# kontera-technologies/redis-bloomfilter

Measured on AMD Instinct MI355X. Metric: keys/sec (insert, include?) per GPU and whole node; % of HBM random-access roofline, higher is better.
Workload: dtype u32

## Files before the change

### redis-bloomfilter_amd/csrc/bf_api.cpp

```cpp
#include "bfhip.h"
#include "bf_host.h"
#include "bf_multi.h"
#include "bf_device.h"

#include <sched.h>

#include <algorithm>
#include <atomic>
#include <cmath>
#include <condition_variable>
#include <functional>
#include <thread>
#include <cstdio>
#include <cstdlib>
#include <cstring>
#include <mutex>
#include <string>
#include <vector>

#define BFHIP_VERSION_STR "bfhip 0.1.0 (gfx950; redis-bloomfilter 1.1.2 ruby-driver layout)"

namespace {

thread_local std::string g_create_error;
// ... 262 lines not shown

int check_keys_args(bf_handle* h, const void* keys, const uint64_t* offsets, uint64_t n) {
    if (!h) return BF_EINVAL;
    if (n == 0) return BF_OK;
    if (!offsets) return set_err(h, BF_EINVAL, "offsets is NULL");
    if (!keys && offsets[n] != offsets[0]) return set_err(h, BF_EINVAL, "key_bytes is NULL");
    return BF_OK;
}

bool binned_pays(const bf_handle* h, uint32_t mode, double probes) {
    if (mode == 0) return false;
    return mode == 1 || (h->dev_bytes >= (64ull << 20) && probes * 128.0 > kBinnedCostRatio * (double)h->dev_bytes);
}

bool use_binned(const bf_handle* h, uint64_t n, bool include, BfBinPlan* plan) {
    if (h->shards > 1 || h->engine != BF_ENGINE_RUBY) return false;
    return binned_pays(h, include ? h->include_binned_mode : h->binned_mode, (double)n * (double)h->k) &&
           bf_binned_plan(h->dev_bytes, n, h->k, h->bin_region_log2, include, plan);
}

int ensure_scratch(bf_handle* h, uint64_t bytes) {
    if (bytes <= h->bin_scratch_cap) return BF_OK;
    (void)hipDeviceSynchronize();
    if (h->d_bin_scratch) (void)hipFree(h->d_bin_scratch);
    h->d_bin_scratch = nullptr;
    h->bin_scratch_cap = 0;
    const uint64_t cap = round_up(bytes, 16ull << 20);
    HIPCHK(h, hipMalloc(&h->d_bin_scratch, cap));
    h->bin_scratch_cap = cap;
    return BF_OK;
}

const char* op_kernel_name(BfOp op) {
    switch (op) {
        case BF_OP_INDEXES: return "bf_keys_kernel<INDEXES>";
        case BF_OP_INCLUDE: return "bf_keys_kernel<INCLUDE>";
        case BF_OP_INSERT: return "bf_keys_kernel<INSERT>";
        case BF_OP_INSERT_FLAGS: return "bf_keys_kernel<INSERT_FLAGS>";
        default: return "bf_keys_kernel<ROUTE>";
    }
}

int launch_op(bf_handle* h, BfOp op, const uint8_t* k16, const uint64_t* offs, uint64_t bias, uint64_t n,
              uint8_t* out8, uint64_t* out64, uint32_t* flag, hipStream_t s) {
    if (h->engine != BF_ENGINE_RUBY) {
        if (op == BF_OP_INSERT_FLAGS && out8)
            return set_err(h, BF_EINVAL, "per_key_new is not available with a RubyTest hash engine");
        if (op == BF_OP_INSERT_FLAGS) op = BF_OP_INSERT;
        BfMarks* mk = prof_begin(h, s);
        HIPCHK(h, bf_launch_engine(h->engine, op, h->g, k16, offs, bias, n, out8, out64, flag, s));
        bf_mark(mk, s, h->engine == BF_ENGINE_MD5 ? "engine_kernel<MD5>" : "engine_kernel<SHA1>");
// ... 469 lines not shown
int bf_destroy(bf_handle* h) {
    if (!h) return BF_OK;
    if (h->multi) {
        bfm_destroy(h->multi);
        delete h;
        return BF_OK;
    }
    {
        CallScope cs(h);
        DeviceGuard dg(h->device);
        if (h->order_valid) (void)hipEventSynchronize(h->order_ev);
        if (h->stream) (void)hipStreamSynchronize(h->stream);
        free_staging(h);
        if (h->h_small) (void)hipHostFree(h->h_small);
        if (h->d_small) (void)hipFree(h->d_small);
        if (h->g.bits) (void)hipFree(h->g.bits);
        if (h->d_flag) (void)hipFree(h->d_flag);
        if (h->d_scan) (void)hipFree(h->d_scan);
        if (h->h_flag) (void)hipHostFree(h->h_flag);
        if (h->h_key_status) (void)hipHostFree(h->h_key_status);
        if (h->d_tmp_local) (void)hipFree(h->d_tmp_local);
        if (h->d_tmp_owner) (void)hipFree(h->d_tmp_owner);
        if (h->d_cursor) (void)hipFree(h->d_cursor);
        if (h->d_bin_scratch) (void)hipFree(h->d_bin_scratch);
        if (h->d_ans8) (void)hipFree(h->d_ans8);
        if (h->d_seg) (void)hipFree(h->d_seg);
        if (h->d_dirty) (void)hipFree(h->d_dirty);
        (void)prof_harvest(h);
        prof_destroy(h);
        if (h->order_ev) (void)hipEventDestroy(h->order_ev);
        if (h->copy_stream) (void)hipStreamDestroy(h->copy_stream);
        if (h->d2h_stream) (void)hipStreamDestroy(h->d2h_stream);
        if (h->stream) (void)hipStreamDestroy(h->stream);
    }
    delete h;
    return BF_OK;
}

int bf_info(const bf_handle* h, uint64_t* m_bits, uint32_t* k, uint64_t* reach_bits, uint64_t* device_bytes) {
    if (h && h->multi) return bfm_info(h->multi, m_bits, k, reach_bits, device_bytes);
    if (!h) return BF_EINVAL;
    if (m_bits) *m_bits = h->m;
    if (k) *k = h->k;
    if (reach_bits) *reach_bits = h->reach;
    if (device_bytes) *device_bytes = h->dev_bytes;
    return BF_OK;
}
// ... 1428 lines not shown
```

### redis-bloomfilter_amd/csrc/bf_binned.hip

```cpp
#include "bf_device.h"
#include "bfhip.h"

#include <algorithm>
#include <cmath>
#include <cstdlib>

using namespace bfdev;

namespace {
__device__ __forceinline__ void stage_store(uint32_t* p, uint32_t v) { __builtin_nontemporal_store(v, p); }
}

namespace {

constexpr int kTile = 1024;
constexpr int kStageVec = 16384 / 16;
constexpr uint32_t kMaxSup = 256;
constexpr uint32_t kMaxOwners = 256;
constexpr uint32_t kChunkBuckets = 512;
constexpr uint32_t kMaxRel = 9;
constexpr uint32_t kMaxBlocks = 512;
constexpr uint32_t kMaxFrontBlocks = 16384;
constexpr uint32_t kGroupBlocks = 64;
constexpr uint32_t kTileProbes = 12288;
// ... 5 lines not shown
constexpr int kChunkPerLane = kBlockProbes / kTile;
constexpr uint32_t kRunsPerPass = 1024;
constexpr uint32_t kMidBuckets = 128;
constexpr uint32_t kMidParts = 2;
constexpr uint32_t kApplyLanes = 1024;
constexpr uint32_t kPipeLanes = 1024;

__device__ __forceinline__ uint32_t block_excl_scan(uint32_t v, uint32_t* s_w, uint32_t* total) {
    const uint32_t lane = threadIdx.x & 63u, wid = threadIdx.x >> 6, nw = blockDim.x >> 6;
    const uint32_t x = wave_incl_scan(v);
    if (lane == 63u) s_w[wid] = x;
    __syncthreads();
    if (wid == 0) {
        const uint32_t s = wave_incl_scan(lane < nw ? s_w[lane] : 0u);
        if (lane < nw) s_w[lane] = s;
    }
    __syncthreads();
    const uint32_t r = (wid ? s_w[wid - 1] : 0u) + x - v;
    if (total) *total = s_w[nw - 1];
    __syncthreads();
    return r;
}

__device__ __forceinline__ void tile_sha1_words(const uint8_t* keys16, const uint64_t* offsets, uint64_t bias,
                                                uint64_t key0, uint32_t tk, uint32_t* key_status, uint64_t* s_off,
                                                uint4* s_stage, uint4& H0, uint4& H1) {
    auto hash = [&](uint64_t first, uint32_t cnt, uint4& Hd) {
        for_key_tile<kTile, kStageVec>(keys16, offsets, bias, first, cnt, s_off, s_stage, key_status,
            [&](auto staged, uint32_t, const uint32_t* src, uint32_t s, uint32_t L) {
                uint32_t H[5];
                sha1_any<decltype(staged)::value>(src, s, L, H);
                Hd = make_uint4(H[0], H[1], H[2], H[3]);
            });
    };
    hash(key0, tk < (uint32_t)kTile ? tk : kTile, H0);
    if (tk > (uint32_t)kTile) hash(key0 + kTile, tk - kTile, H1);
}

template <bool KEYS, int SLOTS, bool DIG = false>
__device__ __forceinline__ void bin_front_body(BfGeom g, const uint8_t* __restrict__ keys16,
                                                          const uint64_t* __restrict__ offsets, uint64_t bias,
                                                          uint64_t n, uint32_t tile_keys, uint32_t tiles_per_block,
                                                          uint32_t sup_log2, uint32_t nsup,
                                                          uint32_t* __restrict__ level1,
                                                          uint32_t* __restrict__ level1_key,
                                                          uint16_t* __restrict__ stab, uint32_t* __restrict__ gcnt,
                                                          uint8_t* __restrict__ out8) {
    __shared__ uint64_t s_off[kTile + 1];
    __shared__ uint4 s_stage[kStageVec + kStageSlackVec];
    __shared__ uint32_t s_cnt[kMaxSup], s_lbase[kMaxSup], s_gcnt[kMaxSup];
    __shared__ uint32_t s_w[16];
    __shared__ uint32_t s_sorted[kTile * SLOTS];
    __shared__ uint32_t s_key[KEYS ? kTile * SLOTS : 1];
    const uint32_t t = threadIdx.x;
    if (t < kMaxSup) {
        s_cnt[t] = 0;
        s_gcnt[t] = 0;
    }
    __syncthreads();
    const uint32_t k = g.k;
    const uint32_t kpl = tile_keys / kTile;
    const uint64_t smask = (1ull << sup_log2) - 1ull;
    const uint64_t ntiles = (n + tile_keys - 1) / tile_keys;
    const uint64_t tb0 = (uint64_t)blockIdx.x * tiles_per_block;
    const uint64_t tb1 = (tb0 + tiles_per_block < ntiles) ? tb0 + tiles_per_block : ntiles;
    for (uint64_t tile = tb0; tile < tb1; ++tile) {
        const uint64_t key0 = tile * tile_keys;
        const uint32_t tk = (uint32_t)((n - key0) < (uint64_t)tile_keys ? (n - key0) : tile_keys);
        uint4 H0 = make_uint4(0, 0, 0, 0), H1 = make_uint4(0, 0, 0, 0);
        if constexpr (DIG) {
            const uint4* dig = reinterpret_cast<const uint4*>(keys16);
            if (t < tk) H0 = dig[key0 + t];
            if (kTile + t < tk) H1 = dig[key0 + kTile + t];
        } else {
            tile_sha1_words(keys16, offsets, bias, key0, tk, g.key_status, s_off, s_stage, H0, H1);
        }
        const bool live0 = t < tk;
        const bool live1 = kpl == 2 && kTile + t < tk;
        if constexpr (KEYS) {
            if (live0) out8[key0 + t] = 1;
            if (live1) out8[key0 + kTile + t] = 1;
        }
        uint32_t tag[SLOTS], loc[SLOTS];
#pragma unroll
        for (int q = 0; q < SLOTS; ++q) {
            const bool second = kpl == 2 && q >= (int)kTwoKeys;
            const uint32_t i = second ? (uint32_t)q - kTwoKeys : (uint32_t)q;
            const bool live = i < k && (second ? live1 : live0);
            tag[q] = 0xFFFFFFFFu;
            loc[q] = 0;
            if (live) {
                const uint4 H = second ? H1 : H0;
                const uint64_t o = probe_offset(g, H.x, H.y, H.z, H.w, i);
                const uint32_t sb = (uint32_t)(o >> sup_log2);
                tag[q] = (sb << 16) | atomicAdd(s_cnt + sb, 1u);
                loc[q] = (uint32_t)(o & smask);
            }
        }
        __syncthreads();
        const uint32_t c = t < kMaxSup ? s_cnt[t] : 0u;
        const uint32_t ex = block_excl_scan(c, s_w, nullptr);
        if (t <= nsup) stab[(uint64_t)t * ntiles + tile] = (uint16_t)ex;
        if (t < kMaxSup) {
            s_lbase[t] = ex;
            s_gcnt[t] += c;
            s_cnt[t] = 0;
        }
        __syncthreads();
#pragma unroll
        for (int q = 0; q < SLOTS; ++q) {
            if (tag[q] != 0xFFFFFFFFu) {
                const uint32_t d = s_lbase[tag[q] >> 16] + (tag[q] & 0xFFFFu);
                s_sorted[d] = loc[q];
                if constexpr (KEYS) {
                    const bool second = kpl == 2 && q >= (int)kTwoKeys;
                    s_key[d] = (uint32_t)(key0 + (second ? kTile + t : t));
                }
            }
        }
        __syncthreads();
        const uint64_t seg = key0 * k;
        const uint32_t tp = tk * k;
        for (uint32_t j = t; j < tp; j += kTile) {
            stage_store(level1 + seg + j, s_sorted[j]);
            if constexpr (KEYS) level1_key[seg + j] = s_key[j];
        }
    }
    if (t < nsup) gcnt[(uint64_t)blockIdx.x * nsup + t] = s_gcnt[t];
}

template <bool DIG>
__global__ __launch_bounds__(kTile) __attribute__((amdgpu_waves_per_eu(8, 8)))
void bin_front_kernel(BfGeom g, const uint8_t* __restrict__ keys16, const uint64_t* __restrict__ offsets,
                      uint64_t bias, uint64_t n, uint32_t tile_keys, uint32_t tiles_per_block, uint32_t sup_log2,
                      uint32_t nsup, uint32_t* __restrict__ level1, uint32_t* __restrict__ level1_key,
                      uint16_t* __restrict__ stab, uint32_t* __restrict__ gcnt, uint8_t* __restrict__ out8) {
    bin_front_body<false, kSlots, DIG>(g, keys16, offsets, bias, n, tile_keys, tiles_per_block, sup_log2, nsup,
                                       level1, level1_key, stab, gcnt, out8);
}

template <bool KEYS, bool DIG = false>
__global__ __launch_bounds__(kTile) void bin_front_wide_kernel(BfGeom g, const uint8_t* __restrict__ keys16,
                                                               const uint64_t* __restrict__ offsets, uint64_t bias,
                                                               uint64_t n, uint32_t tile_keys,
                                                               uint32_t tiles_per_block, uint32_t sup_log2,
                                                               uint32_t nsup, uint32_t* __restrict__ level1,
                                                               uint32_t* __restrict__ level1_key,
                                                               uint16_t* __restrict__ stab, uint32_t* __restrict__ gcnt,
                                                               uint8_t* __restrict__ out8) {
    bin_front_body<KEYS, kWideSlots, DIG>(g, keys16, offsets, bias, n, tile_keys, tiles_per_block, sup_log2, nsup,
                                          level1, level1_key, stab, gcnt, out8);
}

__global__ __launch_bounds__(kTile) __attribute__((amdgpu_waves_per_eu(8, 8)))
void bin_front_wide_dig_kernel(BfGeom g, const uint8_t* __restrict__ keys16, const uint64_t* __restrict__ offsets,
                               uint64_t bias, uint64_t n, uint32_t tile_keys, uint32_t tiles_per_block,
                               uint32_t sup_log2, uint32_t nsup, uint32_t* __restrict__ level1,
                               uint32_t* __restrict__ level1_key, uint16_t* __restrict__ stab,
                               uint32_t* __restrict__ gcnt, uint8_t* __restrict__ out8) {
    bin_front_body<false, kWideSlots, true>(g, keys16, offsets, bias, n, tile_keys, tiles_per_block, sup_log2, nsup,
                                            level1, level1_key, stab, gcnt, out8);
}

__global__ __launch_bounds__(kTile)
void bin_front_keys_kernel(BfGeom g, const uint8_t* __restrict__ keys16, const uint64_t* __restrict__ offsets,
                           uint64_t bias, uint64_t n, uint32_t tile_keys, uint32_t tiles_per_block, uint32_t sup_log2,
                           uint32_t nsup, uint32_t* __restrict__ level1, uint32_t* __restrict__ level1_key,
                           uint16_t* __restrict__ stab, uint32_t* __restrict__ gcnt, uint8_t* __restrict__ out8) {
    bin_front_body<true, kSlots>(g, keys16, offsets, bias, n, tile_keys, tiles_per_block, sup_log2, nsup, level1,
                                 level1_key, stab, gcnt, out8);
}

template <typename Off, bool KEYS>
__device__ __forceinline__ void bin_front_offsets_body(const Off* __restrict__ local, uint64_t count,
                                                       uint32_t tiles_per_block, uint32_t sup_log2, uint32_t nsup,
                                                       uint32_t* __restrict__ level1,
                                                       uint32_t* __restrict__ level1_key,
                                                       uint16_t* __restrict__ stab, uint32_t* __restrict__ gcnt,
                                                       uint64_t bias, const unsigned long long* __restrict__ wcounts,
                                                       uint32_t wstride, uint64_t wcap, uint64_t limit,
                                                       uint8_t* __restrict__ oob_out) {
    __shared__ uint32_t s_cnt[kMaxSup], s_lbase[kMaxSup], s_gcnt[kMaxSup];
    __shared__ uint32_t s_w[16];
    __shared__ uint32_t s_sorted[kTileProbes];
    __shared__ uint16_t s_key[KEYS ? kTileProbes : 1];
    const uint32_t t = threadIdx.x;
    if (t < kMaxSup) {
        s_cnt[t] = 0;
        s_gcnt[t] = 0;
    }
    __syncthreads();
    const uint64_t smask = (1ull << sup_log2) - 1ull;
    const uint64_t ntiles = (count + kTileProbes - 1) / kTileProbes;
    const bool vec_ok = (reinterpret_cast<uintptr_t>(local) & 15u) == 0;
    static_assert(kTileProbes == kTile * kSlots, "a tile is kSlots entries per lane");
    const uint64_t tb0 = (uint64_t)blockIdx.x * tiles_per_block;
    const uint64_t tb1 = (tb0 + tiles_per_block < ntiles) ? tb0 + tiles_per_block : ntiles;
    for (uint64_t tile = tb0; tile < tb1; ++tile) {
        const uint64_t p0 = tile * kTileProbes;
        uint32_t tp = (uint32_t)((count - p0) < (uint64_t)kTileProbes ? (count - p0) : kTileProbes);
        if (wcounts) {
            const uint64_t w = p0 / wcap, i0 = p0 - w * wcap;
            uint64_t live = wcounts[w * wstride];
            if (live > wcap) live = 0;
// ... 32 lines not shown
        __syncthreads();
        const uint32_t c = t < kMaxSup ? s_cnt[t] : 0u;
        const uint32_t ex = block_excl_scan(c, s_w, nullptr);
        if (t <= nsup) stab[(uint64_t)t * ntiles + tile] = (uint16_t)ex;
        if (t < kMaxSup) {
            s_lbase[t] = ex;
            s_gcnt[t] += c;
            s_cnt[t] = 0;
        }
        __syncthreads();
#pragma unroll
        for (int q = 0; q < kSlots; ++q)
            if (tag[q] != 0xFFFFFFFFu) {
                const uint32_t d = s_lbase[tag[q] >> 16] + (tag[q] & 0xFFFFu);
                s_sorted[d] = loc[q];
                if constexpr (KEYS) s_key[d] = (uint16_t)(t * (uint32_t)kSlots + (uint32_t)q);
            }
        __syncthreads();
        for (uint32_t j = t; j < tp; j += kTile) {
            level1[p0 + j] = s_sorted[j];
            if constexpr (KEYS) level1_key[p0 + j] = (uint32_t)p0 + s_key[j];
        }
    }
    if (t < nsup) gcnt[(uint64_t)blockIdx.x * nsup + t] = s_gcnt[t];
}

template <typename Off>
__global__ __launch_bounds__(kTile) __attribute__((amdgpu_waves_per_eu(8, 8)))
void bin_front_offsets_kernel(const Off* __restrict__ local, uint64_t count, uint32_t tiles_per_block,
                              uint32_t sup_log2, uint32_t nsup, uint32_t* __restrict__ level1,
                              uint16_t* __restrict__ stab, uint32_t* __restrict__ gcnt, uint64_t bias,
                              const unsigned long long* __restrict__ wcounts, uint32_t wstride, uint64_t wcap,
                              uint64_t limit) {
    bin_front_offsets_body<Off, false>(local, count, tiles_per_block, sup_log2, nsup, level1, nullptr, stab, gcnt,
                                       bias, wcounts, wstride, wcap, limit, nullptr);
}

template <typename Off>
__global__ __launch_bounds__(kTile) __attribute__((amdgpu_waves_per_eu(8, 8)))
void bin_front_offsets_keys_kernel(const Off* __restrict__ local, uint64_t count,
                                                                       uint32_t tiles_per_block, uint32_t sup_log2,
                                                                       uint32_t nsup, uint32_t* __restrict__ level1,
                                                                       uint32_t* __restrict__ level1_key,
                                                                       uint16_t* __restrict__ stab,
                                                                       uint32_t* __restrict__ gcnt, uint64_t bias,
                                                                       const unsigned long long* __restrict__ wcounts,
                                                                       uint32_t wstride, uint64_t wcap, uint64_t limit,
                                                                       uint8_t* __restrict__ out8) {
    bin_front_offsets_body<Off, true>(local, count, tiles_per_block, sup_log2, nsup, level1, level1_key, stab, gcnt,
                                      bias, wcounts, wstride, wcap, limit, out8);
}

__global__ __launch_bounds__(kMaxBlocks) void bin_group_sum_kernel(const uint32_t* __restrict__ gcnt,
                                                                   uint32_t nblocks, uint32_t nsup, uint32_t nq,
                                                                   uint32_t* __restrict__ gsum) {
    const uint32_t sb = blockIdx.x;
    for (uint32_t w = threadIdx.x; w < nq * kGroupBlocks; w += kMaxBlocks) {
        uint32_t v = w < nblocks ? gcnt[(uint64_t)w * nsup + sb] : 0u;
#pragma unroll
        for (int off = 32; off > 0; off >>= 1) v += (uint32_t)__shfl_xor((int)v, off);
        if ((w & 63u) == 0) gsum[sb * nq + w / kGroupBlocks] = v;
    }
}

constexpr uint32_t kScanPer = 4;
constexpr uint32_t kScanWindows = 1024 * kScanPer;
constexpr uint32_t kLocalScanPer = 4;
constexpr uint32_t kMaxGroups = 1024 * kLocalScanPer;
constexpr uint32_t kMaxWindows = kMaxSup * kMaxGroups;
__global__ __launch_bounds__(1024) void bin_group_scan_kernel(const uint32_t* __restrict__ gsum, uint32_t N,
                                                              uint32_t* __restrict__ base,
                                                              uint32_t* __restrict__ cb_base,
                                                              uint32_t* __restrict__ cb_window,
                                                              uint32_t* __restrict__ cb_start, uint32_t nq,
                                                              unsigned long long* __restrict__ totals) {
    __shared__ uint32_t s_w[16];
    __shared__ uint32_t s_cb[kScanWindows + 1];
    const uint32_t t = threadIdx.x;
    uint32_t v[kScanPer], cv[kScanPer], sum = 0, csum = 0;
#pragma unroll
    for (uint32_t e = 0; e < kScanPer; ++e) {
        const uint32_t w = kScanPer * t + e;
        v[e] = w < N ? gsum[w] : 0u;
        cv[e] = (v[e] + kBlockProbes - 1) / kBlockProbes;
        sum += v[e];
        csum += cv[e];
    }
    uint32_t total, ctotal;
    uint32_t ex = block_excl_scan(sum, s_w, &total);
    uint32_t cex = block_excl_scan(csum, s_w, &ctotal);
#pragma unroll
    for (uint32_t e = 0; e < kScanPer; ++e) {
        const uint32_t w = kScanPer * t + e;
        if (w < N) {
            base[w] = ex;
            cb_base[w] = cex;
            s_cb[w] = cex;
            if (totals && v[e]) atomicAdd(totals + w / nq, (unsigned long long)v[e]);
        }
        ex += v[e];
        cex += cv[e];
    }
    if (t == 0) {
        base[N] = total;
        cb_base[N] = ctotal;
        s_cb[N] = ctotal;
    }
    __syncthreads();
    for (uint32_t blk = t; blk < ctotal; blk += 1024) {
        uint32_t lo = 0, hi = N - 1;
        while (lo < hi) {
            const uint32_t mid = (lo + hi + 1) >> 1;
            if (s_cb[mid] <= blk) lo = mid; else hi = mid - 1;
        }
        cb_window[blk] = lo;
        cb_start[blk] = base[lo] + (blk - s_cb[lo]) * kBlockProbes;
    }
}

__global__ __launch_bounds__(1024) void bin_scan_local_kernel(const uint32_t* __restrict__ gsum, uint32_t nq,
                                                              uint32_t* __restrict__ base,
                                                              uint32_t* __restrict__ cb_base,
                                                              uint32_t* __restrict__ stot) {
    __shared__ uint32_t s_w[16];
    const uint32_t sb = blockIdx.x, t = threadIdx.x;
    uint32_t v[kLocalScanPer], cv[kLocalScanPer], sum = 0, csum = 0;
#pragma unroll
    for (uint32_t e = 0; e < kLocalScanPer; ++e) {
        const uint32_t q = kLocalScanPer * t + e;
        v[e] = q < nq ? gsum[(uint64_t)sb * nq + q] : 0u;
        cv[e] = (v[e] + kBlockProbes - 1) / kBlockProbes;
        sum += v[e];
        csum += cv[e];
    }
    uint32_t total, ctotal;
    uint32_t ex = block_excl_scan(sum, s_w, &total);
    uint32_t cex = block_excl_scan(csum, s_w, &ctotal);
#pragma unroll
    for (uint32_t e = 0; e < kLocalScanPer; ++e) {
        const uint32_t q = kLocalScanPer * t + e;
// ... 1445 lines not shown
                        const uint32_t ri = (uint32_t)(k4[i] - jbase) - a0;
                        if (((av[u] >> (8 * i)) & 0xFFu) && qa + i >= l0 && qa + i < l1 && ri >= b0 && ri < b1)
                            atomicOr(s_bits + ((ri - b0) >> 5), 1u << (ri & 31u));
                    }
                }
            }
        }
        __syncthreads();
        for (uint32_t i = t; i < pw; i += 1024) {
            const bool edge = (w0 + i == 0) || (w0 + i == nw - 1);
            if (edge) atomicOr(out + w0 + i, s_bits[i]);
            else out[w0 + i] = s_bits[i];
        }
        __syncthreads();
    }
}


uint32_t front_form(uint32_t k) { return k <= kTwoKeys ? 0u : (k <= (uint32_t)kSlots ? 1u : 2u); }
uint32_t front_tile_keys(uint32_t k) { return front_form(k) == 0 ? 2 * kTile : kTile; }

uint32_t scan_form(uint32_t nsup, uint32_t ngroups) { return (uint64_t)nsup * ngroups <= kScanWindows ? 0u : 1u; }

uint32_t probe_density(uint64_t probes, uint32_t nbins, uint32_t region_log2) {
    const uint64_t vecs = (uint64_t)nbins << (region_log2 - 7);
    return probes >= vecs ? 2u : (probes >= vecs / 8 ? 1u : 0u);
}

uint32_t apply_form_default(uint32_t density) { return density == 2 ? 1u : 0u; }

bool apply_pipelined(uint32_t density, uint32_t form, uint32_t region_log2, uint32_t nbins, uint32_t grid) {
    return density && form == 1 && region_log2 == 19 && grid && nbins >= 16 * grid;
}

int region_loads(uint64_t probes, uint32_t nbins) { return probes <= (uint64_t)nbins * 4096u ? 2 : 8; }

struct Carve {
    uint32_t *level1, *level1_key, *level2, *level2_key, *gcnt, *gsum, *base, *cb_base, *cb_window, *cb_start;
    uint16_t *stab, *tabs;
    uint8_t* ans2;
    uint2* runs;
    uint16_t* istart;
    uint32_t* stot;
    uint64_t bytes;
};

Carve carve(const BfBinPlan& p, void* at0) {
    Carve c{};
    uint8_t* at = static_cast<uint8_t*>(at0);
    uint64_t off = 0;
    auto take = [&](uint64_t bytes) { uint8_t* q = at ? at + off : nullptr; off += align256(bytes); return q; };
    const uint64_t N = (uint64_t)p.nsup * p.ngroups;
    const bool l1 = !p.chunked;
    c.level1 = l1 ? reinterpret_cast<uint32_t*>(take(p.probes * 4)) : nullptr;
    c.level2 = p.l2test ? nullptr : reinterpret_cast<uint32_t*>(take(p.probes * 4));
    c.level1_key = l1 && p.with_keys ? reinterpret_cast<uint32_t*>(take(p.probes * 4)) : nullptr;
    c.level2_key = p.with_keys && !p.l2test ? reinterpret_cast<uint32_t*>(take(p.probes * 4)) : nullptr;
    c.stab = l1 ? reinterpret_cast<uint16_t*>(take(p.ntiles * (p.nsup + 1) * 2)) : nullptr;
    c.gcnt = l1 ? reinterpret_cast<uint32_t*>(take((uint64_t)p.nblocks * p.nsup * 4)) : nullptr;
    c.gsum = reinterpret_cast<uint32_t*>(take(N * 4));
    c.base = reinterpret_cast<uint32_t*>(take((N + 1) * 4));
    c.cb_base = reinterpret_cast<uint32_t*>(take((N + 1) * 4));
    c.cb_window = reinterpret_cast<uint32_t*>(take(p.max_chunks * 4));
    c.cb_start = reinterpret_cast<uint32_t*>(take(p.max_chunks * 4));
    c.stot = reinterpret_cast<uint32_t*>(take(2 * kMaxSup * 4));
    if (p.l2test) {
        c.runs = reinterpret_cast<uint2*>(take(N * kRunsPerPass * sizeof(uint2)));
        c.istart = reinterpret_cast<uint16_t*>(take(N * kL2MaxParts * sizeof(uint16_t)));
        c.bytes = off;
        return c;
    }
    if (p.chunked)
        c.runs = reinterpret_cast<uint2*>(take(N * kRunsPerPass * sizeof(uint2)));
    c.tabs = reinterpret_cast<uint16_t*>(take(p.max_chunks * ((1ull << p.rel_log2) + 1) * 2));
    if (p.ordered) c.ans2 = take(p.probes + 16);
    c.bytes = off;
    return c;
}

void launch_scan(const BfBinPlan& p, const Carve& c, hipStream_t s) {
    const uint32_t N = p.nsup * p.ngroups;
    if (scan_form(p.nsup, p.ngroups) == 0) {
        hipLaunchKernelGGL(bin_group_scan_kernel, dim3(1), dim3(1024), 0, s, c.gsum, N, c.base, c.cb_base,
                           c.cb_window, c.cb_start, p.ngroups, (unsigned long long*)nullptr);
        return;
    }
    hipLaunchKernelGGL(bin_scan_local_kernel, dim3(p.nsup), dim3(1024), 0, s, c.gsum, p.ngroups, c.base, c.cb_base,
                       c.stot);
    hipLaunchKernelGGL(bin_scan_top_kernel, dim3(1), dim3(1024), 0, s, c.stot, p.nsup, N, c.base, c.cb_base);
    hipLaunchKernelGGL(bin_scan_fill_kernel, dim3((N + 255) / 256), dim3(256), 0, s, c.gsum, N, p.ngroups, c.stot,
                       c.base, c.cb_base, c.cb_window, c.cb_start);
}

hipError_t launch_groups_mid(const BfGeom& g, const BfBinPlan& p, const Carve& c, hipStream_t s, BfMarks* mk) {
    hipLaunchKernelGGL(bin_group_sum_kernel, dim3(p.nsup), dim3(kMaxBlocks), 0, s, c.gcnt, p.nblocks, p.nsup,
                       p.ngroups, c.gsum);
    launch_scan(p, c, s);
    bf_mark(mk, s, "bin_group");
    const uint32_t tiles_per_group = kGroupBlocks * p.tiles_per_block;
    auto mid = [&](auto kernel) {
        hipLaunchKernelGGL(kernel, dim3(mid_grid(p.nsup, p.ngroups)), dim3(kTile), 0, s, c.level1, c.level1_key, c.stab,
                           p.ntiles, p.tile_probes, tiles_per_group, p.nsup, p.ngroups, p.region_log2, p.rel_log2,
                           c.base, c.cb_base, p.max_chunks, c.tabs, c.level2, c.level2_key);
    };
    if (p.with_keys) mid(bin_mid_kernel<true>);
    else mid(bin_mid_kernel<false>);
    bf_mark(mk, s, p.with_keys ? "bin_mid_keys" : "bin_mid");
    return hipGetLastError();
}

hipError_t launch_partition(const BfGeom& g, const BfBinPlan& p, const Carve& c, const uint8_t* keys16,
                            const uint64_t* offsets, uint64_t bias, uint64_t n, uint8_t* out8, hipStream_t s,
                            BfMarks* mk, bool dig = false) {
    const uint32_t sup_log2 = p.region_log2 + p.rel_log2;
    const bool wide = front_form(g.k) == 2;
    auto front = [&](auto kernel) {
        hipLaunchKernelGGL(kernel, dim3(p.nblocks), dim3(kTile), 0, s, g, keys16, offsets, bias, n, p.tile_keys,
                           p.tiles_per_block, sup_log2, p.nsup, c.level1, c.level1_key, c.stab, c.gcnt, out8);
    };
    if (dig) {
        if (p.with_keys) return hipErrorInvalidValue;
        static const bool wide2 = [] {
            const char* e = BF_AB_GETENV("BFHIP_FRONT_WIDE2");
            return !(e && e[0] == '0');
        }();
        if (wide && wide2) front(bin_front_wide_dig_kernel);
        else if (wide) front(bin_front_wide_kernel<false, true>);
        else front(bin_front_kernel<true>);
        bf_mark(mk, s, "bin_front_digest");
        return launch_groups_mid(g, p, c, s, mk);
    }
    if (wide && p.with_keys) front(bin_front_wide_kernel<true>);
    else if (wide) front(bin_front_wide_kernel<false>);
    else if (p.with_keys) front(bin_front_keys_kernel);
    else front(bin_front_kernel<false>);
    bf_mark(mk, s, p.with_keys ? "bin_front_keys" : "bin_front");
    return launch_groups_mid(g, p, c, s, mk);
}

}

namespace {

uint32_t superbins(uint64_t bitset_bytes, uint32_t pref_region_log2);

uint64_t max_tiles(uint64_t bitset_bytes, uint32_t pref_region_log2) {
    const uint32_t nsup = superbins(bitset_bytes, pref_region_log2);
    if (nsup == 0) return 0;
    const uint64_t groups = std::min<uint64_t>(kMaxWindows / nsup, kMaxGroups);
    const uint64_t blocks = std::min<uint64_t>(kMaxFrontBlocks, groups * kGroupBlocks);
    return blocks * kMaxTilesPerBlock;
}

}

uint64_t bf_binned_max_keys(uint32_t k, uint64_t bitset_bytes, uint32_t pref_region_log2) {
    if (k == 0) return 0;
    const uint64_t tile_keys = front_tile_keys(k);
    const uint64_t n = max_tiles(bitset_bytes, pref_region_log2) * tile_keys;
    return std::min<uint64_t>(n, ((1ull << 32) - 1) / k);
// ... 177 lines not shown
}

hipError_t bf_launch_insert_binned_digests(const BfGeom& g, const BfBinPlan& p, uint64_t bitset_bytes,
                                           const uint4* dig, uint64_t n, void* scratch, uint32_t* any_flag,
                                           hipStream_t s, BfMarks* mk) {
    if (n == 0) return hipSuccess;
    if (p.with_keys) return hipErrorInvalidValue;
    const Carve c = carve(p, scratch);
    hipError_t e = launch_partition(g, p, c, reinterpret_cast<const uint8_t*>(dig), nullptr, 0, n, nullptr, s, mk, true);
    if (e != hipSuccess) return e;
    return launch_apply(g, p, c, bitset_bytes, any_flag, s, mk);
}

hipError_t bf_launch_shard_insert_binned(const BfGeom& g, const BfBinPlan& p, uint64_t bitset_bytes,
                                         const void* local, bool route32, uint64_t count, void* scratch,
                                         uint32_t* any_flag, hipStream_t s, BfMarks* mk, uint64_t bias,
                                         const BfWindows& w) {
    if (count == 0) return hipSuccess;
    if (w.counts && (w.cap == 0 || w.cap % kTileProbes)) return hipErrorInvalidValue;
    const Carve c = carve(p, scratch);
    const uint32_t sup_log2 = p.region_log2 + p.rel_log2;
    auto front = [&](auto kernel, auto* offs) {
        hipLaunchKernelGGL(kernel, dim3(p.nblocks), dim3(kTile), 0, s, offs, count, p.tiles_per_block, sup_log2, p.nsup,
                           c.level1, c.stab, c.gcnt, bias, w.counts, w.stride, w.cap, g.limit);
    };
    if (route32) front(bin_front_offsets_kernel<uint32_t>, static_cast<const uint32_t*>(local));
    else front(bin_front_offsets_kernel<uint64_t>, static_cast<const uint64_t*>(local));
    bf_mark(mk, s, "bin_front_offsets");
    hipError_t e = launch_groups_mid(g, p, c, s, mk);
    if (e != hipSuccess) return e;
    return launch_apply(g, p, c, bitset_bytes, any_flag, s, mk);
}

namespace {

hipError_t launch_test(const BfGeom& g, const BfBinPlan& p, const Carve& c, uint64_t bitset_bytes, uint8_t* out8,
                       hipStream_t s, BfMarks* mk) {
    const uint64_t nwords = bitset_bytes / 4;
    auto test = [&](auto kernel, uint32_t lanes) {
        hipLaunchKernelGGL(kernel, dim3(p.nbins), dim3(lanes), 0, s, g.bits, nwords, c.level2, c.level2_key, c.cb_base,
                           c.cb_start, c.tabs, p.max_chunks, p.ngroups, p.rel_log2, out8);
    };
    if (p.region_log2 == 18) test(bin_test_kernel<18, kApplyLanes / 2>, kApplyLanes / 2);
    else if (p.region_log2 == 19) test(bin_test_kernel<19, kApplyLanes>, kApplyLanes);
    else test(bin_test_kernel<20, kApplyLanes>, kApplyLanes);
    bf_mark(mk, s, "bin_test");
    return hipGetLastError();
}

}

hipError_t bf_launch_shard_test_binned(const BfGeom& g, const BfBinPlan& p, uint64_t bitset_bytes,
                                       const void* local, bool route32, uint64_t count, void* scratch, uint8_t* out8,
                                       hipStream_t s, BfMarks* mk, uint64_t bias, const BfWindows& w) {
    if (count == 0) return hipSuccess;
    if (!p.with_keys || !out8) return hipErrorInvalidValue;
    if (w.counts && (w.cap == 0 || w.cap % kTileProbes)) return hipErrorInvalidValue;
    const Carve c = carve(p, scratch);
    const uint32_t sup_log2 = p.region_log2 + p.rel_log2;
    hipError_t e = hipMemsetAsync(out8, 1, count, s);
    if (e != hipSuccess) return e;
    auto front = [&](auto kernel, auto* offs) {
        hipLaunchKernelGGL(kernel, dim3(p.nblocks), dim3(kTile), 0, s, offs, count, p.tiles_per_block, sup_log2, p.nsup,
                           c.level1, c.level1_key, c.stab, c.gcnt, bias, w.counts, w.stride, w.cap, g.limit, out8);
    };
    if (route32) front(bin_front_offsets_keys_kernel<uint32_t>, static_cast<const uint32_t*>(local));
    else front(bin_front_offsets_keys_kernel<uint64_t>, static_cast<const uint64_t*>(local));
    bf_mark(mk, s, "bin_front_offsets_keys");
    if ((e = launch_groups_mid(g, p, c, s, mk)) != hipSuccess) return e;
    return launch_test(g, p, c, bitset_bytes, out8, s, mk);
}

hipError_t bf_launch_include_binned(const BfGeom& g, const BfBinPlan& p, uint64_t bitset_bytes,
                                    const uint8_t* keys16, const uint64_t* offsets, uint64_t bias, uint64_t n,
                                    void* scratch, uint8_t* out8, hipStream_t s, BfMarks* mk) {
    if (n == 0) return hipSuccess;
    if (!p.with_keys || !out8) return hipErrorInvalidValue;
    const Carve c = carve(p, scratch);
    hipError_t e = launch_partition(g, p, c, keys16, offsets, bias, n, out8, s, mk);
    if (e != hipSuccess) return e;
    return launch_test(g, p, c, bitset_bytes, out8, s, mk);
}


namespace {

struct RouteCarve {
    uint32_t *lo1, *key1, *gcnt, *gsum, *base, *cb_base, *cb_window, *cb_start;
    uint8_t* hi1;
    uint16_t* stab;
    uint64_t bytes;
};
// ... 1030 lines not shown
```

### redis-bloomfilter_amd/csrc/bf_internal.h

```cpp
#pragma once
#include <hip/hip_runtime.h>
#include <stdint.h>
#include <cstdlib>

#ifdef BFHIP_AB_KNOBS
#define BF_AB_GETENV(name) std::getenv(name)
#else
#define BF_AB_GETENV(name) ((const char*)nullptr)
#endif

struct BfGeom {
    uint32_t* bits;
    uint64_t  m;
    double    inv_m;
    uint32_t  k;
    uint32_t  nomod;
    uint32_t  mod_f32;
    float     inv_m_f;
    uint32_t  mod_sub;
    uint32_t  shards;
    uint32_t  block_log2;
    double    inv_shards;
    uint32_t  shards_pow2;
    uint32_t  shard_log2;
    uint32_t  first_round;
    uint32_t  next_round;
    uint32_t  route_agg;
    uint32_t  insert_test;
    uint32_t  route32;
    uint8_t*  dirty;
    uint64_t  limit;
    unsigned long long* flips;
    unsigned long long* flip_count;
    uint64_t  flip_cap;
    uint64_t  flip_tag;
    uint32_t* key_status;
};

inline uint32_t bf_mod_sub(uint64_t m, uint64_t vmax) {
    const uint64_t q = vmax / m;
    return q <= 3 ? (uint32_t)q : 0u;
}

inline uint64_t align256(uint64_t x) { return (x + 255) & ~(uint64_t)255; }

constexpr uint32_t kDirtyShiftBits = 19;

struct BfWindows {
    const unsigned long long* counts = nullptr;
    uint32_t stride = 1;
    uint32_t nwin = 1;
    uint64_t cap = 0;
    BfWindows() = default;
    BfWindows(const uint64_t* c, uint32_t s, uint32_t n, uint64_t wcap)
        : counts(reinterpret_cast<const unsigned long long*>(c)), stride(s ? s : 1u), nwin(n), cap(wcap) {}
};

struct BfChunks {
    uint8_t* dir = nullptr;
    uint64_t dir_bytes = 0;
    uint64_t tiles = 0;
    uint32_t S = 1;
    uint32_t sup_log2 = 0;
    uint32_t sub2 = 0;
    uint32_t region_log2 = 19, rel_log2 = 0;
};
bool bf_chunk_geometry(uint64_t shard0_bits, uint32_t nwin, uint32_t pref_region_log2, BfChunks* cg,
                       uint32_t max_buckets = 0 );
// ... 208 lines not shown
```

Baseline: 13.20 billion.

## Fold group-sum and scan into front kernels via last-block tickets

Front binning kernels now publish per-block superbin counts and use atomic tickets in a zeroed scratch header. The last block of each group reduces that group's counts, and the last group runs the window scan in place. This removes the separate group-sum and scan kernel launches when the scan fits in one block. The digest front path also prefetches the next tile's words while the current tile is processed. The trade-offs are extra atomics, fences and serial tail work in the last block, plus a scratch header that must be reset correctly between launches.

New measurement: 13.25 billion (median of 6 runs). Within noise of the previous version (+0.4%).

```diff
diff --git a/redis-bloomfilter_amd/csrc/bf_api.cpp b/redis-bloomfilter_amd/csrc/bf_api.cpp
--- a/redis-bloomfilter_amd/csrc/bf_api.cpp
+++ b/redis-bloomfilter_amd/csrc/bf_api.cpp
@@ -308,11 +308,19 @@
 int ensure_scratch(bf_handle* h, uint64_t bytes) {
     if (bytes <= h->bin_scratch_cap) return BF_OK;
     (void)hipDeviceSynchronize();
-    if (h->d_bin_scratch) (void)hipFree(h->d_bin_scratch);
+    if (h->d_bin_scratch) (void)hipFree(scratch_ticket(h->d_bin_scratch));
     h->d_bin_scratch = nullptr;
     h->bin_scratch_cap = 0;
     const uint64_t cap = round_up(bytes, 16ull << 20);
-    HIPCHK(h, hipMalloc(&h->d_bin_scratch, cap));
+    void* block = nullptr;
+    HIPCHK(h, hipMalloc(&block, kScratchHead + cap));
+    hipError_t ez = hipMemset(block, 0, kScratchHead);
+    if (ez == hipSuccess) ez = hipStreamSynchronize(nullptr);
+    if (ez != hipSuccess) {
+        (void)hipFree(block);
+        return bf_hip_fail(h, ez, "hipMemset(scratch head)");
+    }
+    h->d_bin_scratch = static_cast<uint8_t*>(block) + kScratchHead;
     h->bin_scratch_cap = cap;
     return BF_OK;
 }
@@ -828,7 +836,7 @@
         if (h->d_tmp_local) (void)hipFree(h->d_tmp_local);
         if (h->d_tmp_owner) (void)hipFree(h->d_tmp_owner);
         if (h->d_cursor) (void)hipFree(h->d_cursor);
-        if (h->d_bin_scratch) (void)hipFree(h->d_bin_scratch);
+        if (h->d_bin_scratch) (void)hipFree(scratch_ticket(h->d_bin_scratch));
         if (h->d_ans8) (void)hipFree(h->d_ans8);
         if (h->d_seg) (void)hipFree(h->d_seg);
         if (h->d_dirty) (void)hipFree(h->d_dirty);
diff --git a/redis-bloomfilter_amd/csrc/bf_binned.hip b/redis-bloomfilter_amd/csrc/bf_binned.hip
--- a/redis-bloomfilter_amd/csrc/bf_binned.hip
+++ b/redis-bloomfilter_amd/csrc/bf_binned.hip
@@ -51,6 +51,121 @@
     return r;
 }
 
+constexpr uint32_t kScanPer = 4;
+constexpr uint32_t kScanWindows = 1024 * kScanPer;
+__device__ __forceinline__ void group_scan_body(const uint32_t* gsum, uint32_t N, uint32_t* base, uint32_t* cb_base,
+                                                uint32_t* cb_window, uint32_t* cb_start, uint32_t nq,
+                                                unsigned long long* totals, uint32_t* s_w, uint32_t* s_cb) {
+    const uint32_t t = threadIdx.x;
+    uint32_t v[kScanPer], cv[kScanPer], sum = 0, csum = 0;
+#pragma unroll
+    for (uint32_t e = 0; e < kScanPer; ++e) {
+        const uint32_t w = kScanPer * t + e;
+        v[e] = w < N ? gsum[w] : 0u;
+        cv[e] = (v[e] + kBlockProbes - 1) / kBlockProbes;
+        sum += v[e];
+        csum += cv[e];
+    }
+    uint32_t total, ctotal;
+    uint32_t ex = block_excl_scan(sum, s_w, &total);
+    uint32_t cex = block_excl_scan(csum, s_w, &ctotal);
+#pragma unroll
+    for (uint32_t e = 0; e < kScanPer; ++e) {
+        const uint32_t w = kScanPer * t + e;
+        if (w < N) {
+            base[w] = ex;
+            cb_base[w] = cex;
+            s_cb[w] = cex;
+            if (totals && v[e]) atomicAdd(totals + w / nq, (unsigned long long)v[e]);
+        }
+        ex += v[e];
+        cex += cv[e];
+    }
+    if (t == 0) {
+        base[N] = total;
+        cb_base[N] = ctotal;
+        s_cb[N] = ctotal;
+    }
+    __syncthreads();
+    for (uint32_t blk = t; blk < ctotal; blk += 1024) {
+        uint32_t lo = 0, hi = N - 1;
+        while (lo < hi) {
+            const uint32_t mid = (lo + hi + 1) >> 1;
+            if (s_cb[mid] <= blk) lo = mid; else hi = mid - 1;
+        }
+        cb_window[blk] = lo;
+        cb_start[blk] = base[lo] + (blk - s_cb[lo]) * kBlockProbes;
+    }
+}
+
+struct BfFold {
+    uint32_t* ticket;
+    uint32_t *gsum, *base, *cb_base, *cb_window, *cb_start;
+    uint32_t nq;
+};
+
+__device__ __forceinline__ void fold_acquire() {
+    if (threadIdx.x == 0) {
+        __builtin_amdgcn_fence(__ATOMIC_ACQUIRE, "agent");
+        asm volatile("s_waitcnt vmcnt(0)" ::: "memory");
+    }
+    __syncthreads();
+}
+
+__device__ __forceinline__ void front_fold(const BfFold& f, uint32_t* gcnt, uint32_t nsup, const uint32_t* s_row,
+                                           uint32_t* s_w, uint32_t* s_buf) {
+    static_assert(kTile == 1024, "group_scan_body takes 1024 lanes");
+    static_assert(2 * kScanWindows + 1 <= kTileProbes, "s_buf is a front's sort buffer");
+    static_assert((1 + kScanWindows) * 4 <= kScratchHead, "a ticket per group (at most kScanWindows), and one");
+    const uint32_t t = threadIdx.x;
+    if (t < nsup)
+        __hip_atomic_store(gcnt + (uint64_t)blockIdx.x * nsup + t, s_row[t], __ATOMIC_RELAXED, __HIP_MEMORY_SCOPE_AGENT);
+    if (!f.ticket) return;
+    const uint32_t nq = f.nq, q = blockIdx.x / kGroupBlocks, w0 = q * kGroupBlocks;
+    const uint32_t gs = gridDim.x - w0 < kGroupBlocks ? gridDim.x - w0 : kGroupBlocks;
+    asm volatile("s_waitcnt vmcnt(0)" ::: "memory");
+    __syncthreads();
+    if (t == 0) s_w[0] = __hip_atomic_fetch_add(f.ticket + 1 + q, 1u, __ATOMIC_RELAXED, __HIP_MEMORY_SCOPE_AGENT);
+    __syncthreads();
+    if (s_w[0] != gs - 1) return;
+    fold_acquire();
+    if (t < kMaxSup) s_buf[t] = 0;
+    __syncthreads();
+    constexpr uint32_t kFoldLoads = kGroupBlocks * kMaxSup / kTile;
+    const uint32_t cells = gs * nsup;
+    const uint32_t* rows = gcnt + (uint64_t)w0 * nsup;
+    uint32_t v[kFoldLoads];
+#pragma unroll
+    for (uint32_t u = 0; u < kFoldLoads; ++u) {
+        const uint32_t e = t + u * kTile;
+        v[u] = e < cells ? __hip_atomic_load(rows + e, __ATOMIC_RELAXED, __HIP_MEMORY_SCOPE_AGENT) : 0u;
+    }
+#pragma unroll
+    for (uint32_t u = 0; u < kFoldLoads; ++u) {
+        const uint32_t e = t + u * kTile;
+        if (v[u]) atomicAdd(s_buf + e % nsup, v[u]);
+    }
+    __syncthreads();
+    if (t < nsup) __hip_atomic_store(f.gsum + t * nq + q, s_buf[t], __ATOMIC_RELAXED, __HIP_MEMORY_SCOPE_AGENT);
+    asm volatile("s_waitcnt vmcnt(0)" ::: "memory");
+    __syncthreads();
+    if (t == 0) {
+        __hip_atomic_store(f.ticket + 1 + q, 0u, __ATOMIC_RELAXED, __HIP_MEMORY_SCOPE_AGENT);
+        s_w[0] = __hip_atomic_fetch_add(f.ticket, 1u, __ATOMIC_RELAXED, __HIP_MEMORY_SCOPE_AGENT);
+    }
+    __syncthreads();
+    if (s_w[0] != nq - 1) return;
+    fold_acquire();
+    const uint32_t N = nsup * nq;
+    uint32_t* s_gsum = s_buf;
+    uint32_t* s_cb = s_buf + kScanWindows;
+    for (uint32_t i = t; i < N; i += kTile)
+        s_gsum[i] = __hip_atomic_load(f.gsum + i, __ATOMIC_RELAXED, __HIP_MEMORY_SCOPE_AGENT);
+    __syncthreads();
+    group_scan_body(s_gsum, N, f.base, f.cb_base, f.cb_window, f.cb_start, nq, nullptr, s_w, s_cb);
+    if (t == 0) __hip_atomic_store(f.ticket, 0u, __ATOMIC_RELAXED, __HIP_MEMORY_SCOPE_AGENT);
+}
+
 __device__ __forceinline__ void tile_sha1_words(const uint8_t* keys16, const uint64_t* offsets, uint64_t bias,
                                                 uint64_t key0, uint32_t tk, uint32_t* key_status, uint64_t* s_off,
                                                 uint4* s_stage, uint4& H0, uint4& H1) {
@@ -66,7 +181,7 @@
     if (tk > (uint32_t)kTile) hash(key0 + kTile, tk - kTile, H1);
 }
 
-template <bool KEYS, int SLOTS, bool DIG = false>
+template <bool KEYS, int SLOTS, bool DIG = false, bool FOLD = true, bool PRE = DIG>
 __device__ __forceinline__ void bin_front_body(BfGeom g, const uint8_t* __restrict__ keys16,
                                                           const uint64_t* __restrict__ offsets, uint64_t bias,
                                                           uint64_t n, uint32_t tile_keys, uint32_t tiles_per_block,
@@ -74,7 +189,7 @@
                                                           uint32_t* __restrict__ level1,
                                                           uint32_t* __restrict__ level1_key,
                                                           uint16_t* __restrict__ stab, uint32_t* __restrict__ gcnt,
-                                                          uint8_t* __restrict__ out8) {
+                                                          uint8_t* __restrict__ out8, BfFold fold) {
     __shared__ uint64_t s_off[kTile + 1];
     __shared__ uint4 s_stage[kStageVec + kStageSlackVec];
     __shared__ uint32_t s_cnt[kMaxSup], s_lbase[kMaxSup], s_gcnt[kMaxSup];
@@ -93,11 +208,25 @@
     const uint64_t ntiles = (n + tile_keys - 1) / tile_keys;
     const uint64_t tb0 = (uint64_t)blockIdx.x * tiles_per_block;
     const uint64_t tb1 = (tb0 + tiles_per_block < ntiles) ? tb0 + tiles_per_block : ntiles;
+    uint4 P0 = make_uint4(0, 0, 0, 0), P1 = make_uint4(0, 0, 0, 0);
+    auto prefetch_words = [&](uint64_t tile) {
+        const uint64_t key0 = tile * tile_keys;
+        const uint32_t tk = (uint32_t)((n - key0) < (uint64_t)tile_keys ? (n - key0) : tile_keys);
+        const uint4* dig = reinterpret_cast<const uint4*>(keys16) + key0;
+        if (t < tk) P0 = dig[t];
+        if (kTile + t < tk) P1 = dig[kTile + t];
+    };
+    if constexpr (DIG && PRE) {
+        if (tb0 < tb1) prefetch_words(tb0);
+    }
     for (uint64_t tile = tb0; tile < tb1; ++tile) {
         const uint64_t key0 = tile * tile_keys;
         const uint32_t tk = (uint32_t)((n - key0) < (uint64_t)tile_keys ? (n - key0) : tile_keys);
         uint4 H0 = make_uint4(0, 0, 0, 0), H1 = make_uint4(0, 0, 0, 0);
-        if constexpr (DIG) {
+        if constexpr (DIG && PRE) {
+            H0 = P0;
+            H1 = P1;
+        } else if constexpr (DIG) {
             const uint4* dig = reinterpret_cast<const uint4*>(keys16);
             if (t < tk) H0 = dig[key0 + t];
             if (kTile + t < tk) H1 = dig[key0 + kTile + t];
@@ -126,6 +255,9 @@
                 loc[q] = (uint32_t)(o & smask);
             }
         }
+        if constexpr (DIG && PRE) {
+            if (tile + 1 < tb1) prefetch_words(tile + 1);
+        }
         __syncthreads();
         const uint32_t c = t < kMaxSup ? s_cnt[t] : 0u;
         const uint32_t ex = block_excl_scan(c, s_w, nullptr);
@@ -155,17 +287,21 @@
             if constexpr (KEYS) level1_key[seg + j] = s_key[j];
         }
     }
-    if (t < nsup) gcnt[(uint64_t)blockIdx.x * nsup + t] = s_gcnt[t];
-}
+    if constexpr (FOLD) front_fold(fold, gcnt, nsup, s_gcnt, s_w, s_sorted);
+    else if (t < nsup) gcnt[(uint64_t)blockIdx.x * nsup + t] = s_gcnt[t];
+}
+
+constexpr bool kFoldOffsetsKeys32 = false;
 
 template <bool DIG>
 __global__ __launch_bounds__(kTile) __attribute__((amdgpu_waves_per_eu(8, 8)))
 void bin_front_kernel(BfGeom g, const uint8_t* __restrict__ keys16, const uint64_t* __restrict__ offsets,
                       uint64_t bias, uint64_t n, uint32_t tile_keys, uint32_t tiles_per_block, uint32_t sup_log2,
                       uint32_t nsup, uint32_t* __restrict__ level1, uint32_t* __restrict__ level1_key,
-                      uint16_t* __restrict__ stab, uint32_t* __restrict__ gcnt, uint8_t* __restrict__ out8) {
+                      uint16_t* __restrict__ stab, uint32_t* __restrict__ gcnt, uint8_t* __restrict__ out8,
+                      BfFold fold) {
     bin_front_body<false, kSlots, DIG>(g, keys16, offsets, bias, n, tile_keys, tiles_per_block, sup_log2, nsup,
-                                       level1, level1_key, stab, gcnt, out8);
+                                       level1, level1_key, stab, gcnt, out8, fold);
 }
 
 template <bool KEYS, bool DIG = false>
@@ -176,9 +312,9 @@
                                                                uint32_t nsup, uint32_t* __restrict__ level1,
                                                                uint32_t* __restrict__ level1_key,
                                                                uint16_t* __restrict__ stab, uint32_t* __restrict__ gcnt,
-                                                               uint8_t* __restrict__ out8) {
-    bin_front_body<KEYS, kWideSlots, DIG>(g, keys16, offsets, bias, n, tile_keys, tiles_per_block, sup_log2, nsup,
-                                          level1, level1_key, stab, gcnt, out8);
+                                                               uint8_t* __restrict__ out8, BfFold fold) {
+    bin_front_body<KEYS, kWideSlots, DIG, true, false>(g, keys16, offsets, bias, n, tile_keys, tiles_per_block,
+                                                       sup_log2, nsup, level1, level1_key, stab, gcnt, out8, fold);
 }
 
 __global__ __launch_bounds__(kTile) __attribute__((amdgpu_waves_per_eu(8, 8)))
@@ -186,21 +322,22 @@
                                uint64_t bias, uint64_t n, uint32_t tile_keys, uint32_t tiles_per_block,
                                uint32_t sup_log2, uint32_t nsup, uint32_t* __restrict__ level1,
                                uint32_t* __restrict__ level1_key, uint16_t* __restrict__ stab,
-                               uint32_t* __restrict__ gcnt, uint8_t* __restrict__ out8) {
-    bin_front_body<false, kWideSlots, true>(g, keys16, offsets, bias, n, tile_keys, tiles_per_block, sup_log2, nsup,
-                                            level1, level1_key, stab, gcnt, out8);
+                               uint32_t* __restrict__ gcnt, uint8_t* __restrict__ out8, BfFold fold) {
+    bin_front_body<false, kWideSlots, true, true, false>(g, keys16, offsets, bias, n, tile_keys, tiles_per_block,
+                                                         sup_log2, nsup, level1, level1_key, stab, gcnt, out8, fold);
 }
 
 __global__ __launch_bounds__(kTile)
 void bin_front_keys_kernel(BfGeom g, const uint8_t* __restrict__ keys16, const uint64_t* __restrict__ offsets,
                            uint64_t bias, uint64_t n, uint32_t tile_keys, uint32_t tiles_per_block, uint32_t sup_log2,
                            uint32_t nsup, uint32_t* __restrict__ level1, uint32_t* __restrict__ level1_key,
-                           uint16_t* __restrict__ stab, uint32_t* __restrict__ gcnt, uint8_t* __restrict__ out8) {
+                           uint16_t* __restrict__ stab, uint32_t* __restrict__ gcnt, uint8_t* __restrict__ out8,
+                           BfFold fold) {
     bin_front_body<true, kSlots>(g, keys16, offsets, bias, n, tile_keys, tiles_per_block, sup_log2, nsup, level1,
-                                 level1_key, stab, gcnt, out8);
-}
-
-template <typename Off, bool KEYS>
+                                 level1_key, stab, gcnt, out8, fold);
+}
+
+template <typename Off, bool KEYS, bool FOLD = true>
 __device__ __forceinline__ void bin_front_offsets_body(const Off* __restrict__ local, uint64_t count,
                                                        uint32_t tiles_per_block, uint32_t sup_log2, uint32_t nsup,
                                                        uint32_t* __restrict__ level1,
@@ -208,7 +345,7 @@
                                                        uint16_t* __restrict__ stab, uint32_t* __restrict__ gcnt,
                                                        uint64_t bias, const unsigned long long* __restrict__ wcounts,
                                                        uint32_t wstride, uint64_t wcap, uint64_t limit,
-                                                       uint8_t* __restrict__ oob_out) {
+                                                       uint8_t* __restrict__ oob_out, BfFold fold) {
     __shared__ uint32_t s_cnt[kMaxSup], s_lbase[kMaxSup], s_gcnt[kMaxSup];
     __shared__ uint32_t s_w[16];
     __shared__ uint32_t s_sorted[kTileProbes];
@@ -287,7 +424,8 @@
             if constexpr (KEYS) level1_key[p0 + j] = (uint32_t)p0 + s_key[j];
         }
     }
-    if (t < nsup) gcnt[(uint64_t)blockIdx.x * nsup + t] = s_gcnt[t];
+    if constexpr (FOLD) front_fold(fold, gcnt, nsup, s_gcnt, s_w, s_sorted);
+    else if (t < nsup) gcnt[(uint64_t)blockIdx.x * nsup + t] = s_gcnt[t];
 }
 
 template <typename Off>
@@ -296,9 +434,9 @@
                               uint32_t sup_log2, uint32_t nsup, uint32_t* __restrict__ level1,
                               uint16_t* __restrict__ stab, uint32_t* __restrict__ gcnt, uint64_t bias,
                               const unsigned long long* __restrict__ wcounts, uint32_t wstride, uint64_t wcap,
-                              uint64_t limit) {
+                              uint64_t limit, BfFold fold) {
     bin_front_offsets_body<Off, false>(local, count, tiles_per_block, sup_log2, nsup, level1, nullptr, stab, gcnt,
-                                       bias, wcounts, wstride, wcap, limit, nullptr);
+                                       bias, wcounts, wstride, wcap, limit, nullptr, fold);
 }
 
 template <typename Off>
@@ -311,9 +449,10 @@
                                                                        uint32_t* __restrict__ gcnt, uint64_t bias,
                                                                        const unsigned long long* __restrict__ wcounts,
                                                                        uint32_t wstride, uint64_t wcap, uint64_t limit,
-                                                                       uint8_t* __restrict__ out8) {
-    bin_front_offsets_body<Off, true>(local, count, tiles_per_block, sup_log2, nsup, level1, level1_key, stab, gcnt,
-                                      bias, wcounts, wstride, wcap, limit, out8);
+                                                                       uint8_t* __restrict__ out8, BfFold fold) {
+    bin_front_offsets_body<Off, true, sizeof(Off) != 4 || kFoldOffsetsKeys32>(
+        local, count, tiles_per_block, sup_log2, nsup, level1, level1_key, stab, gcnt, bias, wcounts, wstride, wcap,
+        limit, out8, fold);
 }
 
 __global__ __launch_bounds__(kMaxBlocks) void bin_group_sum_kernel(const uint32_t* __restrict__ gcnt,
@@ -328,8 +467,6 @@
     }
 }
 
-constexpr uint32_t kScanPer = 4;
-constexpr uint32_t kScanWindows = 1024 * kScanPer;
 constexpr uint32_t kLocalScanPer = 4;
 constexpr uint32_t kMaxGroups = 1024 * kLocalScanPer;
 constexpr uint32_t kMaxWindows = kMaxSup * kMaxGroups;
@@ -341,46 +478,7 @@
                                                               unsigned long long* __restrict__ totals) {
     __shared__ uint32_t s_w[16];
     __shared__ uint32_t s_cb[kScanWindows + 1];
-    const uint32_t t = threadIdx.x;
-    uint32_t v[kScanPer], cv[kScanPer], sum = 0, csum = 0;
-#pragma unroll
-    for (uint32_t e = 0; e < kScanPer; ++e) {
-        const uint32_t w = kScanPer * t + e;
-        v[e] = w < N ? gsum[w] : 0u;
-        cv[e] = (v[e] + kBlockProbes - 1) / kBlockProbes;
-        sum += v[e];
-        csum += cv[e];
-    }
-    uint32_t total, ctotal;
-    uint32_t ex = block_excl_scan(sum, s_w, &total);
-    uint32_t cex = block_excl_scan(csum, s_w, &ctotal);
-#pragma unroll
-    for (uint32_t e = 0; e < kScanPer; ++e) {
-        const uint32_t w = kScanPer * t + e;
-        if (w < N) {
-            base[w] = ex;
-            cb_base[w] = cex;
-            s_cb[w] = cex;
-            if (totals && v[e]) atomicAdd(totals + w / nq, (unsigned long long)v[e]);
-        }
-        ex += v[e];
-        cex += cv[e];
-    }
-    if (t == 0) {
-        base[N] = total;
-        cb_base[N] = ctotal;
-        s_cb[N] = ctotal;
-    }
-    __syncthreads();
-    for (uint32_t blk = t; blk < ctotal; blk += 1024) {
-        uint32_t lo = 0, hi = N - 1;
-        while (lo < hi) {
-            const uint32_t mid = (lo + hi + 1) >> 1;
-            if (s_cb[mid] <= blk) lo = mid; else hi = mid - 1;
-        }
-        cb_window[blk] = lo;
-        cb_start[blk] = base[lo] + (blk - s_cb[lo]) * kBlockProbes;
-    }
+    group_scan_body(gsum, N, base, cb_base, cb_window, cb_start, nq, totals, s_w, s_cb);
 }
 
 __global__ __launch_bounds__(1024) void bin_scan_local_kernel(const uint32_t* __restrict__ gsum, uint32_t nq,
@@ -1872,6 +1970,10 @@
 
 uint32_t scan_form(uint32_t nsup, uint32_t ngroups) { return (uint64_t)nsup * ngroups <= kScanWindows ? 0u : 1u; }
 
+bool scan_folded(uint32_t nsup, uint32_t ngroups, bool front_folds) {
+    return front_folds && scan_form(nsup, ngroups) == 0;
+}
+
 uint32_t probe_density(uint64_t probes, uint32_t nbins, uint32_t region_log2) {
     const uint64_t vecs = (uint64_t)nbins << (region_log2 - 7);
     return probes >= vecs ? 2u : (probes >= vecs / 8 ? 1u : 0u);
@@ -1892,12 +1994,14 @@
     uint2* runs;
     uint16_t* istart;
     uint32_t* stot;
+    uint32_t* ticket;
     uint64_t bytes;
 };
 
 Carve carve(const BfBinPlan& p, void* at0) {
     Carve c{};
     uint8_t* at = static_cast<uint8_t*>(at0);
+    c.ticket = at ? scratch_ticket(at) : nullptr;
     uint64_t off = 0;
     auto take = [&](uint64_t bytes) { uint8_t* q = at ? at + off : nullptr; off += align256(bytes); return q; };
     const uint64_t N = (uint64_t)p.nsup * p.ngroups;
@@ -1942,11 +2046,19 @@
                        c.base, c.cb_base, c.cb_window, c.cb_start);
 }
 
-hipError_t launch_groups_mid(const BfGeom& g, const BfBinPlan& p, const Carve& c, hipStream_t s, BfMarks* mk) {
-    hipLaunchKernelGGL(bin_group_sum_kernel, dim3(p.nsup), dim3(kMaxBlocks), 0, s, c.gcnt, p.nblocks, p.nsup,
-                       p.ngroups, c.gsum);
-    launch_scan(p, c, s);
-    bf_mark(mk, s, "bin_group");
+BfFold fold_args(const BfBinPlan& p, const Carve& c, bool front_folds) {
+    return BfFold{scan_folded(p.nsup, p.ngroups, front_folds) ? c.ticket : nullptr, c.gsum, c.base, c.cb_base, c.cb_window,
+                  c.cb_start, p.ngroups};
+}
+
+hipError_t launch_groups_mid(const BfGeom& g, const BfBinPlan& p, const Carve& c, hipStream_t s, BfMarks* mk,
+                             bool front_folds) {
+    if (!scan_folded(p.nsup, p.ngroups, front_folds)) {
+        hipLaunchKernelGGL(bin_group_sum_kernel, dim3(p.nsup), dim3(kMaxBlocks), 0, s, c.gcnt, p.nblocks, p.nsup,
+                           p.ngroups, c.gsum);
+        launch_scan(p, c, s);
+        bf_mark(mk, s, "bin_group");
+    }
     const uint32_t tiles_per_group = kGroupBlocks * p.tiles_per_block;
     auto mid = [&](auto kernel) {
         hipLaunchKernelGGL(kernel, dim3(mid_grid(p.nsup, p.ngroups)), dim3(kTile), 0, s, c.level1, c.level1_key, c.stab,
@@ -1966,7 +2078,8 @@
     const bool wide = front_form(g.k) == 2;
     auto front = [&](auto kernel) {
         hipLaunchKernelGGL(kernel, dim3(p.nblocks), dim3(kTile), 0, s, g, keys16, offsets, bias, n, p.tile_keys,
-                           p.tiles_per_block, sup_log2, p.nsup, c.level1, c.level1_key, c.stab, c.gcnt, out8);
+                           p.tiles_per_block, sup_log2, p.nsup, c.level1, c.level1_key, c.stab, c.gcnt, out8,
+                           fold_args(p, c, true));
     };
     if (dig) {
         if (p.with_keys) return hipErrorInvalidValue;
@@ -1978,14 +2091,14 @@
         else if (wide) front(bin_front_wide_kernel<false, true>);
         else front(bin_front_kernel<true>);
         bf_mark(mk, s, "bin_front_digest");
-        return launch_groups_mid(g, p, c, s, mk);
+        return launch_groups_mid(g, p, c, s, mk, true);
     }
     if (wide && p.with_keys) front(bin_front_wide_kernel<true>);
     else if (wide) front(bin_front_wide_kernel<false>);
     else if (p.with_keys) front(bin_front_keys_kernel);
     else front(bin_front_kernel<false>);
     bf_mark(mk, s, p.with_keys ? "bin_front_keys" : "bin_front");
-    return launch_groups_mid(g, p, c, s, mk);
+    return launch_groups_mid(g, p, c, s, mk, true);
 }
 
 }
@@ -2209,12 +2322,12 @@
     const uint32_t sup_log2 = p.region_log2 + p.rel_log2;
     auto front = [&](auto kernel, auto* offs) {
         hipLaunchKernelGGL(kernel, dim3(p.nblocks), dim3(kTile), 0, s, offs, count, p.tiles_per_block, sup_log2, p.nsup,
-                           c.level1, c.stab, c.gcnt, bias, w.counts, w.stride, w.cap, g.limit);
+                           c.level1, c.stab, c.gcnt, bias, w.counts, w.stride, w.cap, g.limit, fold_args(p, c, true));
     };
     if (route32) front(bin_front_offsets_kernel<uint32_t>, static_cast<const uint32_t*>(local));
     else front(bin_front_offsets_kernel<uint64_t>, static_cast<const uint64_t*>(local));
     bf_mark(mk, s, "bin_front_offsets");
-    hipError_t e = launch_groups_mid(g, p, c, s, mk);
+    hipError_t e = launch_groups_mid(g, p, c, s, mk, true);
     if (e != hipSuccess) return e;
     return launch_apply(g, p, c, bitset_bytes, any_flag, s, mk);
 }
@@ -2247,14 +2360,16 @@
     const uint32_t sup_log2 = p.region_log2 + p.rel_log2;
     hipError_t e = hipMemsetAsync(out8, 1, count, s);
     if (e != hipSuccess) return e;
+    const bool folds = !route32 || kFoldOffsetsKeys32;
     auto front = [&](auto kernel, auto* offs) {
         hipLaunchKernelGGL(kernel, dim3(p.nblocks), dim3(kTile), 0, s, offs, count, p.tiles_per_block, sup_log2, p.nsup,
-                           c.level1, c.level1_key, c.stab, c.gcnt, bias, w.counts, w.stride, w.cap, g.limit, out8);
+                           c.level1, c.level1_key, c.stab, c.gcnt, bias, w.counts, w.stride, w.cap, g.limit, out8,
+                           fold_args(p, c, folds));
     };
     if (route32) front(bin_front_offsets_keys_kernel<uint32_t>, static_cast<const uint32_t*>(local));
     else front(bin_front_offsets_keys_kernel<uint64_t>, static_cast<const uint64_t*>(local));
     bf_mark(mk, s, "bin_front_offsets_keys");
-    if ((e = launch_groups_mid(g, p, c, s, mk)) != hipSuccess) return e;
+    if ((e = launch_groups_mid(g, p, c, s, mk, folds)) != hipSuccess) return e;
     return launch_test(g, p, c, bitset_bytes, out8, s, mk);
 }
 
diff --git a/redis-bloomfilter_amd/csrc/bf_internal.h b/redis-bloomfilter_amd/csrc/bf_internal.h
--- a/redis-bloomfilter_amd/csrc/bf_internal.h
+++ b/redis-bloomfilter_amd/csrc/bf_internal.h
@@ -44,6 +44,11 @@
 
 inline uint64_t align256(uint64_t x) { return (x + 255) & ~(uint64_t)255; }
 
+constexpr uint64_t kScratchHead = 16640;
+inline uint32_t* scratch_ticket(void* scratch) {
+    return reinterpret_cast<uint32_t*>(static_cast<uint8_t*>(scratch) - kScratchHead);
+}
+
 constexpr uint32_t kDirtyShiftBits = 19;
 
 struct BfWindows {
```
